# guenthermi/postgres-word2vec

Measured on AMD Instinct MI355X. Metric: batched IVFADC kNN queries/sec (k=5) + recall@5, 3Mx300d, higher is better.
Workload: dtype f32; 1 GPU; IVFADC batch (ivfadc_batch_search generalised to nprobe), 3000000x300d, C=1000, m=12, K=1024, nprobe=10, k=5, batch=1024 queries per GPU, replicated index, queries sharded by rank; N=3000000, d=300, C=1000, m=12, K=1024, nprobe=10, k=5, batch_per_gpu=1024, parallelism=dp1, world_size=1, backend=none (single GPU), batches_in_flight=4

## Files before the change

### postgres-word2vec_amd/csrc/fused5.h

```cpp
#pragma once
#include <hip/hip_runtime.h>
#include <stdint.h>

#include "refine.h"
#include "coarse.h"
#include "scan_tail5.h"

namespace freddy {

static constexpr int SCAN5_G = 16;

__host__ __device__ __forceinline__ constexpr int filt5_bias(int p, int m) { return FILT5_VMAX + (p < 32768 - FILT5_VMAX * m ? 1 : 0); }
__device__ __forceinline__ uint32_t lane_byte4() {
  uint32_t x;
  asm volatile("v_mbcnt_lo_u32_b32 %0, -1, 0\n\tv_mbcnt_hi_u32_b32 %0, -1, %0\n\tv_lshlrev_b32 %0, 2, %0" : "=v"(x));
  return x;
}
typedef short s2v __attribute__((ext_vector_type(2)));
__device__ __forceinline__ uint32_t pk_add_i16(uint32_t x, uint32_t y) {
  return __builtin_bit_cast(uint32_t, __builtin_bit_cast(s2v, x) + __builtin_bit_cast(s2v, y));
}

template <int S, int QT>
__device__ __forceinline__ void query_codebook5_body(const float* __restrict__ queries, const float* __restrict__ cbT,
                                                     const float* __restrict__ cmax, float* __restrict__ qn,
                                                     float* __restrict__ qscale, uint32_t* __restrict__ qc,
                                                     int Q, int d, int m, int K, int bx, int by, unsigned char* smem,
                                                     uint32_t* __restrict__ qc8 = nullptr) {
  static_assert(QT == 16, "one 16-lane group per query");
  constexpr int SP = (S + 3) & ~3;
  float (*qs)[SP] = reinterpret_cast<float (*)[SP]>(smem);
  float* inv_s = reinterpret_cast<float*>(smem + QT * SP * 4);
  const int tid = threadIdx.x, p = bx, q0 = by * QT;
  constexpr int STEPS_B = (S + 3) / 4;
  float bv[STEPS_B][4][2];
  auto load_b = [&](int g) {
    typedef float f4b __attribute__((ext_vector_type(4)));
    const f4b* src = reinterpret_cast<const f4b*>(cbT + ((((size_t)p * 8 + g) * STEPS_B) * 64 + (tid & 63)) * 8);
#pragma unroll
    for (int st = 0; st < STEPS_B; ++st) {
      const f4b lo = src[(size_t)st * 128], hi = src[(size_t)st * 128 + 1];
      bv[st][0][0] = lo.x; bv[st][0][1] = lo.y; bv[st][1][0] = lo.z; bv[st][1][1] = lo.w;
      bv[st][2][0] = hi.x; bv[st][2][1] = hi.y; bv[st][3][0] = hi.z; bv[st][3][1] = hi.w;
    }
  };
  load_b((tid >> 6) * 2);
  for (int i = tid; i < QT * SP; i += 256) {
    const int qi = i / SP, j = i - qi * SP;
    qs[qi][j] = (j < S && q0 + qi < Q) ? queries[(size_t)(q0 + qi) * d + p * S + j] : 0.0f;
  }
  {
    const int qi = tid >> 4, pp = tid & 15, q = q0 + qi;
    float best = 0.0f;
    if (pp < m && q < Q) {
      float n2 = 0.0f;
      for (int j = 0; j < S; ++j) { const float v = queries[(size_t)q * d + pp * S + j]; n2 = __builtin_fmaf(v, v, n2); }
      const float nrm = __builtin_sqrtf(n2) * (1.0f + 1e-5f);
      if (p == 0) qn[(size_t)q * m + pp] = nrm;
      best = 2.0f * nrm * cmax[pp];
    }
#pragma unroll
    for (int o = 8; o > 0; o >>= 1) best = fmaxf(best, __shfl_xor(best, o, 64));
    if (pp == 0) {
      const float sc = q < Q ? best * (1.0f / (float)FILT5_VMAX) * (1.0f + 1e-6f) : 0.0f;
      inv_s[qi] = (sc > 0.0f && sc < 1e30f) ? 1.0f / sc : 0.0f;
      if (p == 0 && q < Q) qscale[q] = sc;
    }
  }
  {
    typedef float f4v __attribute__((ext_vector_type(4)));
    __syncthreads();
    const int wave = tid >> 6, lane = tid & 63, col = lane & 15, kq = lane >> 4;
    const int nq = (Q - q0 < QT) ? Q - q0 : QT;
    constexpr int STEPS = (S + 3) / 4;
    float av[STEPS];
#pragma unroll
    for (int st = 0; st < STEPS; ++st) av[st] = 4 * st + kq < S ? qs[col][4 * st + kq] : 0.0f;
    const float vmax = (float)FILT5_VMAX;
    const int bias = filt5_bias(p, m);
#pragma unroll
    for (int gg = 0; gg < 2; ++gg) {
      const int g = wave * 2 + gg;
      f4v acc[4][2];
#pragma unroll
      for (int i = 0; i < 4; ++i) acc[i][0] = acc[i][1] = f4v{0.0f, 0.0f, 0.0f, 0.0f};
#pragma unroll
      for (int st = 0; st < STEPS; ++st)
#pragma unroll
        for (int i = 0; i < 4; ++i)
#pragma unroll
          for (int e = 0; e < 2; ++e) acc[i][e] = __builtin_amdgcn_mfma_f32_16x16x4f32(av[st], bv[st][i][e], acc[i][e], 0, 0, 0);
      if (gg == 0) load_b(g + 1);
#pragma unroll
      for (int reg = 0; reg < 4; ++reg) {
        const int qi = 4 * kq + reg;
        if (qi < nq) {
          const float inv = inv_s[qi];
          uint32_t wd[4];
#pragma unroll
          for (int i = 0; i < 4; ++i) {
            const int i0 = (int)fminf(fmaxf(__builtin_rintf(-2.0f * acc[i][0][reg] * inv), -vmax), vmax) + bias;
            const int i1 = (int)fminf(fmaxf(__builtin_rintf(-2.0f * acc[i][1][reg] * inv), -vmax), vmax) + bias;
            wd[i] = (uint32_t)i0 | ((uint32_t)i1 << 16);
          }
          *reinterpret_cast<uint4*>(qc + ((size_t)(q0 + qi) * m + p) * 512 + 4 * (16 * g + col)) = uint4{wd[0], wd[1], wd[2], wd[3]};
          if (qc8) qc8[((size_t)(q0 + qi) * m + p) * 128 + (16 * g + col)] = (wd[0] & 0xffffu) | (wd[1] << 16);
        }
      }
    }
  }
}
template <int S, int QT>
static constexpr int query_codebook5_lds() { return QT * ((S + 3) & ~3) * 4 + QT * 4; }
template <int S, int QT>
__global__ __launch_bounds__(256) void query_codebook5_kernel(const float* __restrict__ queries, const float* __restrict__ cbT,
                                                             const float* __restrict__ cmax, float* __restrict__ qn,
                                                             float* __restrict__ qscale, uint32_t* __restrict__ qc,
                                                             int Q, int d, int m, int K, uint32_t* __restrict__ qc8) {
  __shared__ __attribute__((aligned(16))) unsigned char smem[query_codebook5_lds<S, QT>()];
  query_codebook5_body<S, QT>(queries, cbT, cmax, qn, qscale, qc, Q, d, m, K, blockIdx.x, blockIdx.y, smem, qc8);
}

struct CoarseTableArgs {
  const float* queries;
  const float* coarseF; const float* cn2; float* dist; float* qn2; int Q, Cpad, d, dp; ZeroArgs z; int coarse_gx, coarse_gy;
  const float* cbT; const float* cmax; float* qn; float* qscale; uint32_t* qc; int m, K;
  float* tmin; int C;
  const ch8v* coarseH; int ec;
  uint32_t* qc8;
};
template <int S, int QT, bool H16 = false>
__global__ __launch_bounds__(256) void coarse_table5_kernel(CoarseTableArgs a) {
  extern __shared__ __attribute__((aligned(16))) unsigned char smem[];
  const int n_coarse = a.coarse_gx * a.coarse_gy;
  const int b = blockIdx.x;
  if (b < n_coarse) {
    if constexpr (H16)
      coarse_approx16_body(a.queries, a.coarseH, a.ec, a.cn2, a.dist, a.qn2, a.Q, a.Cpad, a.d, a.z, b % a.coarse_gx, b / a.coarse_gx,
                           a.coarse_gx, a.coarse_gy, smem, a.tmin, a.C);
    else
    coarse_approx_body(a.queries, a.coarseF, a.cn2, a.dist, a.qn2, a.Q, a.Cpad, a.d, a.dp, a.z, b % a.coarse_gx, b / a.coarse_gx,
                       a.coarse_gx, a.coarse_gy, smem, a.tmin, a.C);
  } else {
    const int t = b - n_coarse;
    query_codebook5_body<S, QT>(a.queries, a.cbT, a.cmax, a.qn, a.qscale, a.qc, a.Q, a.d, a.m, a.K, t % a.m, t / a.m, smem, a.qc8);
  }
}

template <int M>
__global__ __launch_bounds__(256) void entry_record5_kernel(RecordArgs a) {
  const int lane = threadIdx.x & 63;
  const int e = blockIdx.x * 4 + (threadIdx.x >> 6);
  if (a.elastic && blockIdx.x == 0 && threadIdx.x == 0) __hip_atomic_fetch_add(a.elastic + EL_PENDING, a.n_announce, FREDDY_RLX_AGENT);
  if (e >= a.n_groups[0]) return;
  const int cell = a.group_cell[e], first = a.group_first[e], gc = a.group_cnt[e];
  const int cnt = gc & 0xff, chunk = gc >> 8;
  int32_t* rec = a.records + (size_t)e * REC_DW;
  if (lane == 0) {
    const int b0 = a.blk_off[cell] + chunk * FUSED_UNIT_BLOCKS;
    int nb = a.blk_off[cell + 1] - b0;
    if (nb > FUSED_UNIT_BLOCKS) nb = FUSED_UNIT_BLOCKS;
    int rows = a.list_off[cell + 1] - a.list_off[cell] - chunk * (FUSED_UNIT_BLOCKS * 64);
    if (rows > FUSED_UNIT_BLOCKS * 64) rows = FUSED_UNIT_BLOCKS * 64;
    rec[0] = cell; rec[1] = cnt; rec[2] = chunk; rec[3] = b0; rec[4] = nb; rec[5] = rows;
  }
  if (lane < 16) {
    const int it = lane < cnt ? a.sorted_item[first + lane] : -1;
    const int q = a.item_query[it >= 0 ? it : a.sorted_item[first]];
    const float sc = a.qscale[q];
    ItemBounds ib = item_bounds(0.0f, 0.0f, a.sentinel);
    if (it >= 0) ib = item_bounds(a.item_dist[it], filter_width5<M>(a.qn + (size_t)q * M, a.pmax, sc), a.sentinel);
    rec[8 + lane] = it;
    rec[24 + lane] = q;
    rec[40 + lane] = (int32_t)__float_as_uint(ib.off);
    rec[56 + lane] = (int32_t)__float_as_uint(ib.e);
    rec[72 + lane] = (int32_t)__float_as_uint(ib.shift);
    rec[88 + lane] = (int32_t)ib.lo_bits;
    rec[104 + lane] = (int32_t)ib.hi_bits;
    rec[128 + lane] = (int32_t)__float_as_uint((it >= 0 && sc < 1e30f) ? sc : 0.0f);
    const float A = it >= 0 ? a.item_dist[it] : -1.0f;
    const bool fin = it >= 0 && ib.e < 1e30f && A >= 0.0f && A < 1e30f;
    rec[144 + lane] = (int32_t)__float_as_uint(fin ? A * (1.0f + 2e-5f) : __uint_as_float(0x7f800000u));
    rec[160 + lane] = (int32_t)__float_as_uint(fin ? A * (1.0f - 2e-5f) : 0.0f);
  }
}

template <int M, bool FULLK, bool CAND, bool PROF, bool U8, bool ELASTIC>
__device__ __forceinline__ void ivf_filter5_body(const FilterArgs& a) {
  static_assert(!(U8 && FULLK), "one byte per code: K <= 256");
  constexpr int G = SCAN5_G, RMAX = FUSED_RMAX, NG = SPEC2_NG;
  constexpr int NP = M / 2;
  constexpr int ROWB = G * 2;
  constexpr int HROWB = 16;
  static_assert(M == 12 && G == 16 && SPEC2_NB == 8, "layout");
  typedef uint32_t u2 __attribute__((ext_vector_type(2)));
  typedef uint32_t u4 __attribute__((ext_vector_type(4)));
  extern __shared__ __attribute__((aligned(16))) unsigned char smem[];
  unsigned char* slab = smem;
  uint32_t* colmin = reinterpret_cast<uint32_t*>(smem + a.desc_offset);
  uint32_t* thr_s = colmin + 16 * 64;
  int32_t* dsc = reinterpret_cast<int32_t*>(smem + a.desc_offset + 4096 + 64);
  int32_t* gidq = dsc + 2 * REC_DW;
  float* rt_s = reinterpret_cast<float*>(gidq + 4);

  const int tid = threadIdx.x, lane = tid & 63;
  const int wave = __builtin_amdgcn_readfirstlane(tid >> 6);
  const bool builder = wave < SPEC2_NB;
  const int K = FULLK ? 1024 : a.K;
  const uint32_t HALFB = (uint32_t)K * HROWB;
  const uint32_t POSB = 2u * HALFB;
  const uint32_t BUFB = 2u * POSB;
  const int n_work = a.n_groups[0];

  int cur = 0, ei = 0;
  const int n_own = ELASTIC ? a.n_own : (int)gridDim.x;
  const bool extra = ELASTIC && (int)blockIdx.x >= n_own;
  if (!extra) {
    if (tid == 0) {
      gidq[0] = (int)blockIdx.x; gidq[1] = n_own + atomicAdd(a.work_counter, 1);
      if constexpr (ELASTIC) {
        __hip_atomic_fetch_sub(a.elastic + EL_PENDING, 1, FREDDY_RLX_AGENT);
        if ((int)blockIdx.x < n_work) __hip_atomic_fetch_add(a.elastic + EL_ACTIVE, 1, FREDDY_RLX_AGENT);
      }
    }
    if (tid < REC_DW) dsc[tid] = a.records[(size_t)blockIdx.x * REC_DW + tid];
  } else if (tid == 0) {
    const int pend = __hip_atomic_load(a.elastic + EL_PENDING, FREDDY_RLX_AGENT);
    const int claims = __hip_atomic_load(a.work_counter, FREDDY_RLX_AGENT);
    const int alive = __hip_atomic_fetch_add(a.elastic + EL_ACTIVE, 1, FREDDY_RLX_AGENT);
    int g = -1;
    if (pend - (claims < n_own ? n_own - claims : 0) <= 0 && alive < a.cap) g = n_own + atomicAdd(a.work_counter, 1);
    if (g < 0 || g >= n_work) {
      g = -1;
      __hip_atomic_fetch_sub(a.elastic + EL_ACTIVE, 1, FREDDY_RLX_AGENT);
    } else {
      __hip_atomic_fetch_add(a.elastic + EL_STARTED, 1, FREDDY_RLX_AGENT);
    }
    const bool leave = g >= 0 && a.elastic_yield == 2;
    if (leave) __hip_atomic_fetch_add(a.elastic + EL_YIELDED, 1, FREDDY_RLX_AGENT);
    gidq[0] = g; gidq[1] = (leave || g < 0) ? 0x7fffffff : n_own + atomicAdd(a.work_counter, 1); gidq[2] = leave ? 1 : 0;
  }
  for (int i = tid; i < 16 * 64; i += SPEC2_T) colmin[i] = 0xffffffffu;
  __syncthreads();
  if (extra) {
    const int first = __builtin_amdgcn_readfirstlane(gidq[0]);
    if (first < 0) return;
    if (tid < REC_DW) dsc[tid] = a.records[(size_t)first * REC_DW + tid];
    __syncthreads();
  } else if ((int)blockIdx.x >= n_work) return;

  if (builder) {
    const int hpos = (wave >> 1) & 1;
    const int half = wave >> 2;
    const int li = (wave & 1) * 64 + lane;
    const uint32_t qoff = (uint32_t)hpos * POSB + (uint32_t)half * HALFB + (uint32_t)li * HROWB;
    const uint32_t vq = (uint32_t)li * 16u + (uint32_t)hpos * 2048u;
    u4 qw[2][8];
#pragma unroll
    for (int s = 0; s < 2; ++s)
#pragma unroll
      for (int g = 0; g < 8; ++g) qw[s][g] = u4{0u, 0u, 0u, 0u};
    typedef const char __attribute__((address_space(1))) * gptrc;
    typedef const u4 __attribute__((address_space(1))) * gptr4u;
    auto issue = [&](int set, int phase, const int (&qids)[8], int nh) {
      if (half >= nh || (a.fence & 32)) return;
      uint32_t voff = vq + (uint32_t)phase * 4096u;
      asm volatile("" : "+v"(voff));
#pragma unroll
      for (int u = 0; u < 8; ++u) {
        const gptrc qb = (gptrc)(uintptr_t)a.qc + (size_t)(uint32_t)qids[u] * (size_t)(M * 2048);
        qw[set][u] = *(gptr4u)(qb + voff);
      }
    };
    auto emit = [&](int set, unsigned char* dst, int nh) {
      if (half >= nh || (a.fence & 16)) return;
      unsigned char* dp = dst + qoff;
#pragma unroll
      for (int k = 0; k < 4; ++k) {
        uint32_t w[8];
#pragma unroll
        for (int u = 0; u < 8; ++u)
          w[u] = k == 0 ? qw[set][u].x : k == 1 ? qw[set][u].y : k == 2 ? qw[set][u].z : qw[set][u].w;
        const u4 lo = u4{__builtin_amdgcn_perm(w[1], w[0], 0x05040100u), __builtin_amdgcn_perm(w[3], w[2], 0x05040100u),
                         __builtin_amdgcn_perm(w[5], w[4], 0x05040100u), __builtin_amdgcn_perm(w[7], w[6], 0x05040100u)};
        const u4 hi = u4{__builtin_amdgcn_perm(w[1], w[0], 0x07060302u), __builtin_amdgcn_perm(w[3], w[2], 0x07060302u),
// ... 265 lines not shown
```

### postgres-word2vec_amd/csrc/pin.hip

```cpp
#include "internal.h"

#include "kernels.h"
#include "scan_common.h"
#include "coarse.h"
#include "mutate.h"

static std::vector<float> transpose_codebook(const float* cb, int m, int K, int S) {
  std::vector<float> t((size_t)m * S * K);
  for (int p = 0; p < m; ++p)
    for (int c = 0; c < K; ++c)
      for (int j = 0; j < S; ++j) t[((size_t)p * S + j) * K + c] = cb[((size_t)p * K + c) * S + j];
  return t;
}

static void arrange_list_rows(const int16_t* codes, int m, int64_t lo, int64_t hi, std::vector<int64_t>& order) {
  const int64_t n = hi - lo;
  order.resize((size_t)n);
  for (int64_t i = 0; i < n; ++i) order[(size_t)i] = lo + i;
  if (n <= 16 || m > 16) return;
  static const int WINDOW = (int)env_int("FREDDY_GPU_ARRANGE_WINDOW", 1024);
  int cnt[16][16], mx[16];
  for (int64_t k = 0; k < n; ++k) {
    if ((k & 15) == 0) { memset(cnt, 0, sizeof(cnt)); memset(mx, 0, sizeof(mx)); }
    const int64_t wend = std::min<int64_t>(n, k + WINDOW);
    int64_t best = k;
    int best_cost = INT32_MAX;
    for (int64_t j = k; j < wend; ++j) {
      const int16_t* row = codes + (size_t)order[(size_t)j] * m;
      int cost = 0;
      for (int p = 0; p < m; ++p) {
        const int c = cnt[p][row[p] & 15];
        cost += c + (c + 1 > mx[p] ? 100 : 0);
      }
      if (cost < best_cost) { best_cost = cost; best = j; }
    }
    std::swap(order[(size_t)k], order[(size_t)best]);
    const int16_t* row = codes + (size_t)order[(size_t)k] * m;
    for (int p = 0; p < m; ++p) {
      const int c = ++cnt[p][row[p] & 15];
      if (c > mx[p]) mx[p] = c;
    }
  }
  static const int GROUP_LANES[64] = {0,  1,  2,  3,  12, 13, 14, 15, 20, 21, 22, 23, 24, 25, 26, 27, 4,  5,  6,  7,  8,  9,
                                      10, 11, 16, 17, 18, 19, 28, 29, 30, 31, 32, 33, 34, 35, 44, 45, 46, 47, 52, 53, 54, 55,
                                      56, 57, 58, 59, 36, 37, 38, 39, 40, 41, 42, 43, 48, 49, 50, 51, 60, 61, 62, 63};
  std::vector<int64_t> blk(64);
  for (int64_t b0 = 0; b0 + 64 <= n; b0 += 64) {
    for (int j = 0; j < 64; ++j) blk[(size_t)GROUP_LANES[j]] = order[(size_t)(b0 + j)];
    for (int j = 0; j < 64; ++j) order[(size_t)(b0 + j)] = blk[(size_t)j];
  }
}

static int pack_lists(freddy_gpu_index* ix, int n_lists, const int32_t* list_off, const int16_t* codes,
                      const int32_t* row_pos ) {
  const int m = ix->m, K = ix->K, M2 = ix->M2;
  BlockPlan plan;
  int bad = 0;
  if (const int why = plan_blocks(n_lists, [&](int c) { return (int64_t)list_off[c + 1] - list_off[c]; }, plan, &bad))
    return why == PLAN_NEGATIVE_LENGTH ? fail(FREDDY_E_ARG, "list_off is not non-decreasing at list %d", bad) : fail(FREDDY_E_LIMIT, "N too large for 32-bit row positions");
  const std::vector<int32_t>& blk_off = plan.blk_off;
  const int64_t n_blocks = plan.n_blocks;
  std::vector<uint32_t> packed((size_t)alloc_blocks(n_blocks) * M2 * 64, 0u);
  std::vector<int32_t> pos((size_t)alloc_blocks(n_blocks) * 64, -1);
  const bool arrange = row_pos != nullptr;
  std::vector<std::vector<int64_t>> orders(arrange ? (size_t)n_lists : 0);
  if (arrange) {
    std::atomic<int> next_list{0};
    auto worker = [&]() {
      for (int c = next_list.fetch_add(1); c < n_lists; c = next_list.fetch_add(1))
        arrange_list_rows(codes, m, list_off[c], list_off[c + 1], orders[(size_t)c]);
    };
    const unsigned nt = std::max(1u, std::min(32u, std::thread::hardware_concurrency()));
    std::vector<std::thread> pool;
    for (unsigned t = 1; t < nt && (int)t < n_lists; ++t) pool.emplace_back(worker);
    worker();
    for (auto& th : pool) th.join();
  }
  for (int c = 0; c < n_lists; ++c) {
    for (int64_t i = 0; i < (int64_t)list_off[c + 1] - list_off[c]; ++i) {
      const int64_t r = arrange ? orders[(size_t)c][(size_t)i] : list_off[c] + i;
      const int64_t b = blk_off[c] + i / 64;
      const int lane = (int)(i % 64);
      const int16_t* row = codes + (size_t)r * m;
      for (int l = 0; l < m; ++l) {
        if (row[l] < 0 || row[l] >= K)
          return fail(FREDDY_E_ARG, "code %d at row %lld position %d is outside [0,%d)", (int)row[l],
                      (long long)r, l, K);
      }
      for (int j = 0; j < M2; ++j) {
        const uint32_t lo = (uint16_t)row[2 * j];
        const uint32_t hi = (2 * j + 1 < m) ? (uint16_t)row[2 * j + 1] : 0u;
        packed[((size_t)b * M2 + j) * 64 + lane] = lo | (hi << 16);
      }
      pos[(size_t)b * 64 + lane] = row_pos ? row_pos[r] : (int32_t)r;
    }
  }
  if (upload(&ix->blk_cell, plan.blk_cell.data(), plan.blk_cell.size(), &ix->bytes))
    return fail(FREDDY_E_NOMEM, "device allocation/copy failed while pinning the lists");
  ix->n_blocks = n_blocks;
  ix->max_list_blocks = plan.max_list_blocks;
  ix->h_list_off.assign(list_off, list_off + n_lists + 1);
  if (upload(&ix->blk_off, blk_off.data(), blk_off.size(), &ix->bytes) ||
      upload(&ix->list_off, list_off, (size_t)n_lists + 1, &ix->bytes) ||
      upload(&ix->packed, packed.data(), packed.size(), &ix->bytes) ||
      upload(&ix->pos, pos.data(), pos.size(), &ix->bytes))
    return fail(FREDDY_E_NOMEM, "device allocation/copy failed while pinning the lists");
  return 0;
}

__global__ __launch_bounds__(256) void pack8_kernel(const uint32_t* __restrict__ packed, uint32_t* __restrict__ packed8, int64_t n_blocks) {
  const int64_t i = (int64_t)blockIdx.x * 256 + threadIdx.x;
  if (i >= n_blocks * 3 * 64) return;
  const int lane = (int)(i & 63);
  const int64_t bt = i >> 6;
  const int t = (int)(bt % 3);
  const int64_t b = bt / 3;
  const uint32_t p0 = packed[((size_t)b * 6 + 2 * t) * 64 + lane], p1 = packed[((size_t)b * 6 + 2 * t + 1) * 64 + lane];
  packed8[i] = (p0 & 0xffu) | (((p0 >> 16) & 0xffu) << 8) | ((p1 & 0xffu) << 16) | (((p1 >> 16) & 0xffu) << 24);
}
static int make_packed8(const freddy_gpu_index* ix, const uint32_t* packed, int64_t n_blocks, uint32_t** out, int64_t* out_bytes) {
  *out = nullptr; *out_bytes = 0;
  if (ix->K > 256 || ix->m != 12 || ix->M2 != 6 || !packed || n_blocks <= 0) return 0;
  const size_t bytes = sizeof(uint32_t) * (size_t)n_blocks * 3 * 64;
  if (dev_malloc(out, bytes) != hipSuccess) { *out = nullptr; return fail(FREDDY_E_NOMEM, "device allocation of %zu bytes failed (one-byte codes)", bytes); }
  const int64_t n = n_blocks * 3 * 64;
  hipLaunchKernelGGL(pack8_kernel, dim3((unsigned)((n + 255) / 256)), dim3(256), 0, ix->stream, packed, *out, n_blocks);
  if (hipGetLastError() != hipSuccess || hipStreamSynchronize(ix->stream) != hipSuccess) {
    (void)dev_free(*out); *out = nullptr;
    return fail(FREDDY_E_HIP, "building the one-byte codes failed");
  }
  *out_bytes = (int64_t)bytes;
  return 0;
}
static void install_packed8(freddy_gpu_index* ix, uint32_t* p8, int64_t bytes) {
  if (ix->packed8 && ix->packed8_own) { (void)dev_free(ix->packed8); ix->bytes -= ix->packed8_bytes; }
  ix->packed8 = p8; ix->packed8_own = p8 != nullptr; ix->packed8_bytes = bytes;
  ix->bytes += bytes;
}
static int build_packed8(freddy_gpu_index* ix) {
  uint32_t* p8 = nullptr;
  int64_t bytes = 0;
  if (int rc = make_packed8(ix, ix->packed, ix->n_blocks, &p8, &bytes)) return rc;
  install_packed8(ix, p8, bytes);
  return 0;
}

static int derive_codebook_tables_into(freddy_gpu_index* ix, const float* codebook);
static int make_row_terms(const freddy_gpu_index* ix, const uint32_t* packed, const int32_t* blk_cell, int64_t n_blocks, const float* cbR, float** out, int64_t* out_bytes);
static void install_row_terms(freddy_gpu_index* ix, float* rterm, int64_t bytes);
static int derive_codebook_tables(freddy_gpu_index* ix, const float* codebook, bool with_row_terms = false) {
  float* const old[] = {ix->cbT, ix->cbP, ix->cbR, ix->pmax, ix->cmaxp, ix->cbF};
  const int64_t bytes_before = ix->bytes;
  ix->cbT = ix->cbP = ix->cbR = ix->pmax = ix->cmaxp = ix->cbF = nullptr;
  int rc = derive_codebook_tables_into(ix, codebook);
  float* rterm = nullptr;
  int64_t rterm_bytes = 0;
  if (!rc && with_row_terms) rc = make_row_terms(ix, ix->packed, ix->blk_cell, ix->n_blocks, ix->cbR, &rterm, &rterm_bytes);
  if (rc) {
    float* const fresh[] = {ix->cbT, ix->cbP, ix->cbR, ix->pmax, ix->cmaxp, ix->cbF};
    for (float* p : fresh) if (p) (void)dev_free(p);
    ix->cbT = old[0]; ix->cbP = old[1]; ix->cbR = old[2]; ix->pmax = old[3]; ix->cmaxp = old[4]; ix->cbF = old[5];
    ix->bytes = bytes_before;
    return rc;
  }
  if (with_row_terms) install_row_terms(ix, rterm, rterm_bytes);
  int64_t old_bytes = 0;
  if (old[0]) old_bytes += (int64_t)sizeof(float) * ix->m * ix->S * ix->K;
  if (old[1]) old_bytes += (int64_t)sizeof(float) * ix->m * (((ix->S + 3) & ~3) / 4) * FUSED_T * 8;
  if (old[2]) old_bytes += (int64_t)sizeof(float) * ix->m * ix->K * ix->S;
  if (old[3]) old_bytes += (int64_t)sizeof(float) * ix->m;
  if (old[4]) old_bytes += (int64_t)sizeof(float) * ix->m;
  if (old[5]) old_bytes += (int64_t)sizeof(float) * ix->m * 8 * 7 * 64 * 8;
  ix->bytes -= old_bytes;
  for (float* p : old) if (p) (void)dev_free(p);
  if (ix->kind == KIND_PQ) drop_pq_views(ix);
  return 0;
}
static int build_fragment_codebook(freddy_gpu_index* ix, const float* codebook) {
  std::vector<float> f((size_t)ix->m * 8 * 7 * 64 * 8, 0.0f);
  for (int p = 0; p < ix->m; ++p)
    for (int g = 0; g < 8; ++g)
      for (int st = 0; st < 7; ++st)
        for (int l = 0; l < 64; ++l)
          for (int i = 0; i < 4; ++i)
            for (int e = 0; e < 2; ++e) {
              const int j = 4 * st + (l >> 4), c = 128 * i + 16 * g + (l & 15) + 512 * e;
              if (j < ix->S && c < ix->K)
                f[((((size_t)p * 8 + g) * 7 + st) * 64 + l) * 8 + i * 2 + e] = codebook[((size_t)p * ix->K + c) * ix->S + j];
            }
  if (upload(&ix->cbF, f.data(), f.size(), &ix->bytes)) return fail(FREDDY_E_NOMEM, "device allocation failed");
  return 0;
}
static inline double norm_max(double a, double b) { return (b != b || b > a) ? b : a; }
static int derive_codebook_tables_into(freddy_gpu_index* ix, const float* codebook) {
  std::vector<float> cbT = transpose_codebook(codebook, ix->m, ix->K, ix->S);
  if (upload(&ix->cbT, cbT.data(), cbT.size(), &ix->bytes)) return fail(FREDDY_E_NOMEM, "device allocation failed");
  if (ix->kind == KIND_PQ) {
    if (ix->m == 12 && ix->S == 25 && ix->K <= FUSED_T * FUSED_E) {
      std::vector<float> cmaxp((size_t)ix->m);
      for (int p = 0; p < ix->m; ++p) {
        double cmax = 0.0;
        for (int c = 0; c < ix->K; ++c) {
          double n2 = 0.0;
          for (int j = 0; j < ix->S; ++j) { const double v = codebook[((size_t)p * ix->K + c) * ix->S + j]; n2 += v * v; }
          cmax = norm_max(cmax, std::sqrt(n2));
        }
        cmaxp[p] = (float)(cmax * (1.0 + 1e-6));
      }
      if (upload(&ix->cbR, codebook, (size_t)ix->m * ix->K * ix->S, &ix->bytes) ||
          upload(&ix->pmax, cmaxp.data(), cmaxp.size(), &ix->bytes) ||
          upload(&ix->cmaxp, cmaxp.data(), cmaxp.size(), &ix->bytes))
        return fail(FREDDY_E_NOMEM, "device allocation failed");
      if (int rc = build_fragment_codebook(ix, codebook)) return rc;
    }
    return 0;
  }
  if (ix->kind != KIND_IVF) return 0;
  const int C = ix->C, d = ix->d;
  if (ix->K <= FUSED_T * FUSED_E) {
    const int SP = (ix->S + 3) & ~3, SPq = SP / 4;
    std::vector<float> cbP((size_t)ix->m * SPq * FUSED_T * 8, 0.0f);
    for (int p = 0; p < ix->m; ++p)
      for (int jb = 0; jb < SPq; ++jb)
        for (int tl = 0; tl < FUSED_T; ++tl)
          for (int u = 0; u < 4; ++u)
            for (int e = 0; e < 2; ++e) {
              const int j = jb * 4 + u, c = tl + e * FUSED_T;
              if (j < ix->S && c < ix->K)
                cbP[((((size_t)p * SPq + jb) * FUSED_T + tl) * 4 + u) * 2 + e] = codebook[((size_t)p * ix->K + c) * ix->S + j];
            }
    if (upload(&ix->cbP, cbP.data(), cbP.size(), &ix->bytes)) return fail(FREDDY_E_NOMEM, "device allocation failed");
  }
  if (ix->cbP && ix->m == 12 && ix->S == 25) {
    std::vector<float> pmax((size_t)ix->m), cmaxp((size_t)ix->m);
    for (int p = 0; p < ix->m; ++p) {
      double comax = 0.0, cmax = 0.0;
      for (int c = 0; c < C; ++c) {
        double n2 = 0.0;
        for (int j = 0; j < ix->S; ++j) { const double v = ix->h_coarse[(size_t)c * d + p * ix->S + j]; n2 += v * v; }
        comax = norm_max(comax, std::sqrt(n2));
      }
      for (int c = 0; c < ix->K; ++c) {
        double n2 = 0.0;
        for (int j = 0; j < ix->S; ++j) { const double v = codebook[((size_t)p * ix->K + c) * ix->S + j]; n2 += v * v; }
        cmax = norm_max(cmax, std::sqrt(n2));
      }
      pmax[p] = (float)((comax + cmax) * (1.0 + 1e-6));
      cmaxp[p] = (float)(cmax * (1.0 + 1e-6));
    }
    if (upload(&ix->cbR, codebook, (size_t)ix->m * ix->K * ix->S, &ix->bytes) ||
        upload(&ix->pmax, pmax.data(), pmax.size(), &ix->bytes) ||
        upload(&ix->cmaxp, cmaxp.data(), cmaxp.size(), &ix->bytes))
      return fail(FREDDY_E_NOMEM, "device allocation failed");
    if (int rc = build_fragment_codebook(ix, codebook)) return rc;
  }
  return 0;
}

static int make_row_terms(const freddy_gpu_index* ix, const uint32_t* packed, const int32_t* blk_cell, int64_t n_blocks, const float* cbR, float** out, int64_t* out_bytes) {
  *out = nullptr; *out_bytes = 0;
  if (!cbR) return 0;
  const int64_t n_slots = alloc_blocks(n_blocks) * 64;
  if (dev_malloc(out, sizeof(float) * (size_t)n_slots) != hipSuccess) { *out = nullptr; return fail(FREDDY_E_NOMEM, "device allocation failed (row terms)"); }
  if (n_blocks > 0) {
    hipLaunchKernelGGL(row_term_kernel, dim3((unsigned)((n_blocks * 64 + 255) / 256)), dim3(256), 0, ix->stream, packed,
                       blk_cell, ix->coarse, cbR, *out, n_blocks * 64, ix->M2, ix->d, ix->m, ix->K, ix->S);
    if (hipGetLastError() != hipSuccess || hipStreamSynchronize(ix->stream) != hipSuccess) {
      (void)dev_free(*out); *out = nullptr;
      return fail(FREDDY_E_HIP, "building the row terms failed");
    }
  }
  *out_bytes = (int64_t)sizeof(float) * n_slots;
  return 0;
}
static void install_row_terms(freddy_gpu_index* ix, float* rterm, int64_t bytes) {
  if (ix->rterm) (void)dev_free(ix->rterm);
  ix->bytes += bytes - ix->rterm_bytes;
  ix->rterm = rterm; ix->rterm_bytes = bytes;
}
static int refresh_row_terms(freddy_gpu_index* ix) {
  float* rterm = nullptr;
  int64_t bytes = 0;
  if (int rc = make_row_terms(ix, ix->packed, ix->blk_cell, ix->n_blocks, ix->cbR, &rterm, &bytes)) return rc;
  install_row_terms(ix, rterm, bytes);
  return 0;
}

static int raise_lds_limits(int device) {
  static std::mutex mu;
  static std::vector<char> done;
  std::lock_guard<std::mutex> g(mu);
  if ((size_t)device < done.size() && done[(size_t)device]) return 0;
  for (const std::vector<LdsLimit>& unit : {lds_limits_ivfadc(), lds_limits_pq(), lds_limits_join(), lds_limits_exact()})
    for (const LdsLimit& l : unit) HIP_TRY(hipFuncSetAttribute(l.kernel, hipFuncAttributeMaxDynamicSharedMemorySize, l.bytes));
  if (done.size() <= (size_t)device) done.resize((size_t)device + 1, 0);
  done[(size_t)device] = 1;
  return 0;
}

int open_device(freddy_gpu_index* ix, int device) {
  if (!ix->registered) { ix->registered = true; backend_handles(+1, device); }
  choose_hw_queues(device);
  int n = 0;
  HIP_TRY(hipGetDeviceCount(&n));
  if (device < 0 || device >= n) return fail(FREDDY_E_ARG, "device %d out of range (%d visible)", device, n);
  HIP_TRY(hipSetDevice(device));
  ix->device = device;
  ix->tune = read_tuning();
  if (int rc = raise_lds_limits(device)) return rc;
  HIP_TRY(hipStreamCreateWithFlags(&ix->stream, hipStreamNonBlocking));
  hipDeviceProp_t prop;
  if (hipGetDeviceProperties(&prop, device) == hipSuccess && prop.multiProcessorCount > 0) ix->n_cus = ix->device_cus = prop.multiProcessorCount;
  return 0;
}

static int check_pq_shape(int d, int m, int K, int64_t N) {
  if (d <= 0 || m <= 0 || K <= 0 || N < 0) return fail(FREDDY_E_ARG, "non-positive dimension");
  if (d % m) return fail(FREDDY_E_ARG, "d=%d is not a multiple of m=%d", d, m);
  if (K > 65536) return fail(FREDDY_E_LIMIT, "K=%d does not fit a 16-bit code", K);
  if ((size_t)m * K * 4 + 4096 > 160 * 1024)
    return fail(FREDDY_E_LIMIT, "LUT of m*K=%d floats does not fit the 160 KiB LDS", m * K);
  if (N > (int64_t)INT32_MAX - 64) return fail(FREDDY_E_LIMIT, "N too large for 32-bit row positions");
  return 0;
}

extern "C" int freddy_gpu_pin_pq(const freddy_pq_desc* t, int device, freddy_gpu_index_t** out) {
  if (!t || !out || !t->codebook || (t->N && (!t->ids || !t->codes))) return fail(FREDDY_E_ARG, "NULL argument");
  if (int rc = check_pq_shape(t->d, t->m, t->K, t->N)) return rc;
  for (int64_t r = 1; r < t->N; ++r)
    if (t->ids[r] <= t->ids[r - 1])
      return fail(FREDDY_E_ARG, "ids must be strictly ascending (canonical scan order); violated at row %lld", (long long)r);
  freddy_gpu_index* ix = new freddy_gpu_index();
  ix->kind = KIND_PQ;
  ix->d = t->d; ix->m = t->m; ix->K = t->K; ix->S = t->d / t->m; ix->M2 = (t->m + 1) / 2; ix->N = t->N;
  int rc = open_device(ix, device);
  if (!rc) rc = derive_codebook_tables(ix, t->codebook);
  if (!rc && upload(&ix->ids, t->ids, (size_t)t->N, &ix->bytes)) rc = fail(FREDDY_E_NOMEM, "device allocation failed");
  if (!rc) {
    const int32_t off[2] = {0, (int32_t)t->N};
    rc = pack_lists(ix, 1, off, t->codes, nullptr);
    if (!rc) rc = build_packed8(ix);
  }
  if (!rc) { ix->h_ids.assign(t->ids, t->ids + t->N); ix->max_id = t->N ? t->ids[t->N - 1] : -1; }
// ... 147 lines not shown
```

### postgres-word2vec_amd/csrc/refine.h

```cpp
#pragma once
#include <hip/hip_runtime.h>
#include <stdint.h>

#include "scan_common.h"
#include "fused3.h"

namespace freddy {

struct FilterArgs {
  const uint32_t* qc;
  const float* rterm;
  const int32_t* records;
  const int32_t* n_groups;
  int32_t* work_counter;
  const uint32_t* packed;
  u64* surv;
  int32_t* surv_count;
  int32_t* cand_count;
  int K, L, upi;
  float sentinel;
  uint32_t desc_offset;
  uint32_t fence;
  int keep_all;
  long long* prof;
  const uint32_t* packed8;
  uint32_t* tau_run;
  const uint32_t* qc8;
  int Lt;
  int32_t* elastic;
  int n_own, cap, elastic_yield;
};
enum { EL_ACTIVE = 0, EL_PENDING = 1, EL_STARTED = 2, EL_YIELDED = 3 };
#define FREDDY_RLX_AGENT __ATOMIC_RELAXED, __HIP_MEMORY_SCOPE_AGENT

static constexpr int FILT5_VMAX = 2730;
static constexpr float FILT5_EPS = 512.0f * 5.9604644775390625e-8f * 1.0001f;
template <int M>
__device__ __forceinline__ float filter_width5(const float* __restrict__ qn, const float* __restrict__ pmax, float scale) {
  float sb = 0.0f;
#pragma unroll
  for (int p = 0; p < M; ++p) {
    const float t = qn[p] + pmax[p];
    sb = __builtin_fmaf(t, t, sb);
  }
  return __builtin_fmaf(sb, FILT5_EPS, __builtin_fmaf(28.0f, scale, 1e-30f));
}

struct ItemBounds {
  float off;
  float e;
  float shift;
  uint32_t lo_bits;
  uint32_t hi_bits;
};
__device__ __forceinline__ ItemBounds item_bounds(float A, float E, float sentinel) {
  ItemBounds b;
  if (E < 1e30f && A < 1e30f && A >= 0.0f) {
    const float a_up = A * (1.0f + 2e-5f), a_lo = A * (1.0f - 2e-5f);
    b.off = a_up + E;
    b.e = E;
    b.shift = ((b.off - a_lo) + 0.25f * E) * (1.0f + 1e-6f);
    const float hi = (sentinel + b.shift) * (1.0f + 1e-6f);
    const float lo = ((sentinel + b.shift) - E) * (1.0f - 1e-6f);
    b.hi_bits = hi < 3e38f ? __float_as_uint(hi) : 0xfffffffeu;
    b.lo_bits = lo > 0.0f ? __float_as_uint(lo < 3e38f ? lo : 3e38f) : 0u;
  } else {
    b.off = 0.0f;
    b.e = __uint_as_float(0x7f800000u);
    b.shift = __uint_as_float(0x7f800000u);
    b.lo_bits = 0u;
    b.hi_bits = 0xfffffffeu;
  }
  return b;
}
__device__ __forceinline__ uint32_t widen_threshold(uint32_t tau_bits, float E) {
  if (tau_bits >= 0x7f800000u || !(E < 1e30f)) return 0xfffffffeu;
  const float t = (__uint_as_float(tau_bits) + E) * (1.0f + 2.4e-7f);
  return __float_as_uint(t);
}

static __global__ __launch_bounds__(256) void row_term_kernel(const uint32_t* __restrict__ packed, const int32_t* __restrict__ blk_cell,
                                                      const float* __restrict__ coarse, const float* __restrict__ cbR,
                                                      float* __restrict__ rterm, int64_t n_slots, int M2, int d, int m, int K, int S) {
  const int64_t slot = (int64_t)blockIdx.x * 256 + threadIdx.x;
  if (slot >= n_slots) return;
  const int64_t block = slot >> 6;
  const int lane = (int)(slot & 63);
  const int cell = blk_cell[block];
  double acc = 0.0;
  for (int p = 0; p < m; ++p) {
    const uint32_t word = packed[((size_t)block * M2 + (p >> 1)) * 64 + lane];
    const int code = (int)((word >> ((p & 1) * 16)) & 0xffffu);
    const float* cv = cbR + ((size_t)p * K + (code < K ? code : 0)) * S;
    const float* co = coarse + (size_t)cell * d + (size_t)p * S;
    for (int j = 0; j < S; ++j) acc += (double)cv[j] * (double)cv[j] + 2.0 * (double)co[j] * (double)cv[j];
  }
  rterm[slot] = (float)acc;
}

static constexpr int REC_DW = 176;

struct RecordArgs {
  const int32_t* group_cell;
  const int32_t* group_first;
  const int32_t* group_cnt;
  const int32_t* n_groups;
  const int32_t* sorted_item;
  const int32_t* item_query;
  const int32_t* blk_off;
  const int32_t* list_off;
  const float* item_dist;
  const float* qn;
  const float* qscale;
  const float* pmax;
  int32_t* records;
  float sentinel;
  int32_t* elastic;
  int n_announce;
};

struct MergeRefineArgs {
  const u64* surv;
  const int32_t* surv_count;
  const int32_t* active;
  const int32_t* round_rows;
  const int32_t* item_cell;
  const float* queries;
  const float* coarse;
  const float* cbR;
  const float* qn;
  const float* pmax;
  const float* qscale5;
  const uint32_t* packed;
  const int32_t* pos;
  const int32_t* blk_cell;
  int32_t* cand_count;
  int32_t* violations;
  int32_t* out_ids;
  float* out_dist;
  int32_t* found;
  int32_t* next_active;
  int32_t* n_next;
  int32_t* status;
  int n_active, W, upi, L, k, found_rule, first_round, K, d;
  float sentinel;
  int refine_all;
  uint32_t fence;
  int slices;
  u64* part;
};

template <int S, int M, int NWV, bool MANY = false, bool PARTIAL = false>
__global__ __launch_bounds__(64 * NWV, 4) void merge_refine_kernel(MergeRefineArgs a) {
  static_assert(!MANY || NWV > 1, "the split selection needs the four waves");
  static_assert(!PARTIAL || MANY, "slices of a query: the flat PQ table's instantiation");
  constexpr int NT = NWV > 4 ? NWV : 4;
  static_assert(NT * 64 / M <= 64, "a round's rows are finalised by one wave");
  constexpr int NC = NT * 64 / M;
  constexpr int SQ = S + 1;
  constexpr int M2 = M / 2;
  __shared__ u64 stage_all[MANY ? NWV : 1][64];
  u64* const stage = stage_all[0];
  __shared__ u64 part_key[MANY ? NWV : 1][MANY ? 64 : 1];
  __shared__ uint32_t part_flag[MANY ? NWV : 1][MANY ? 64 : 1];
  __shared__ float qs[M * S];
  __shared__ float sq[NWV == 1 ? 32 * SQ : NT * 64 * SQ];
  __shared__ float lutv[NT * 64];
  __shared__ int32_t cbo[NT * 64], coo[NT * 64];
  __shared__ u64 cq_key[64 + NC];
  __shared__ int32_t cq_cell[64 + NC];
  __shared__ int sh_n;
  constexpr int BQ = MANY ? 512 : 1;
  __shared__ u64 bq_key[BQ];
  constexpr int PB = 256;
  __shared__ int pref_all[MANY ? NWV : 1][PB + 1];
  __shared__ int bq_n;
  __shared__ uint32_t sh_T;
  const int x = blockIdx.x, lane = threadIdx.x & 63;
  const int wave = __builtin_amdgcn_readfirstlane((int)(threadIdx.x >> 6));
  const int q = PARTIAL ? x / a.slices : (a.active ? a.active[x] : x);
  const int k = a.k;
  const int per_item = a.upi * FUSED_NW;
  const int R = a.W * per_item;
  constexpr int NBATCH = 4;

  if (!(a.fence & 2)) for (int j = threadIdx.x; j < M * S; j += 64 * NWV) qs[j] = a.queries[(size_t)q * a.d + j];
  const float E = (a.fence & 2) ? 0.0f : filter_width5<M>(a.qn + (size_t)q * M, a.pmax, a.qscale5[q]);

  auto tile_work = [&](int t, float* sqb, int n) {
// ... 362 lines not shown
```

Measured before the change: 11.99 million queries/s.

## Compute query-codebook table with split-fp16 MFMA instead of fp32 MFMA

Replaces the fp32 16x16x4 MFMA loop (7 k-steps per output tile) in the query-codebook table kernel with three 16x16x32 fp16 MFMAs per tile. Queries and codebook are each split into hi and lo fp16 parts with per-position power-of-two exponent scaling, and the results are unscaled with ldexp. The host-side fragment codebook is rebuilt as hi/lo fp16 halves with stored exponents. It also adds a waves_per_eu(4) occupancy hint to the table kernels. The aim is fewer matrix instructions and less codebook load traffic, at the cost of dropping the lo*lo term, which could slightly perturb the quantized table values.

```diff
diff --git a/postgres-word2vec_amd/csrc/fused5.h b/postgres-word2vec_amd/csrc/fused5.h
--- a/postgres-word2vec_amd/csrc/fused5.h
+++ b/postgres-word2vec_amd/csrc/fused5.h
@@ -32,19 +32,15 @@
   float (*qs)[SP] = reinterpret_cast<float (*)[SP]>(smem);
   float* inv_s = reinterpret_cast<float*>(smem + QT * SP * 4);
   const int tid = threadIdx.x, p = bx, q0 = by * QT;
-  constexpr int STEPS_B = (S + 3) / 4;
-  float bv[STEPS_B][4][2];
+  static_assert(S <= 32 && SP % 4 == 0, "one k-step of v_mfma_f32_16x16x32_f16 covers a position");
+  ch8v bh[8], bl[8];
   auto load_b = [&](int g) {
-    typedef float f4b __attribute__((ext_vector_type(4)));
-    const f4b* src = reinterpret_cast<const f4b*>(cbT + ((((size_t)p * 8 + g) * STEPS_B) * 64 + (tid & 63)) * 8);
-#pragma unroll
-    for (int st = 0; st < STEPS_B; ++st) {
-      const f4b lo = src[(size_t)st * 128], hi = src[(size_t)st * 128 + 1];
-      bv[st][0][0] = lo.x; bv[st][0][1] = lo.y; bv[st][1][0] = lo.z; bv[st][1][1] = lo.w;
-      bv[st][2][0] = hi.x; bv[st][2][1] = hi.y; bv[st][3][0] = hi.z; bv[st][3][1] = hi.w;
-    }
+    const ch8v* src = reinterpret_cast<const ch8v*>(cbT) + ((size_t)p * 8 + g) * (CBF_GROUP_HALVES / 8) + (tid & 63);
+#pragma unroll
+    for (int t = 0; t < 8; ++t) { bh[t] = src[(size_t)t * 128]; bl[t] = src[(size_t)t * 128 + 64]; }
   };
   load_b((tid >> 6) * 2);
+  const int ecb = reinterpret_cast<const int*>(cbT)[cbf_exp_offset(m) + p];
   for (int i = tid; i < QT * SP; i += 256) {
     const int qi = i / SP, j = i - qi * SP;
     qs[qi][j] = (j < S && q0 + qi < Q) ? queries[(size_t)(q0 + qi) * d + p * S + j] : 0.0f;
@@ -72,10 +68,30 @@
     __syncthreads();
     const int wave = tid >> 6, lane = tid & 63, col = lane & 15, kq = lane >> 4;
     const int nq = (Q - q0 < QT) ? Q - q0 : QT;
-    constexpr int STEPS = (S + 3) / 4;
-    float av[STEPS];
-#pragma unroll
-    for (int st = 0; st < STEPS; ++st) av[st] = 4 * st + kq < S ? qs[col][4 * st + kq] : 0.0f;
+    ch8v ah, al;
+    int eq = 0;
+    {
+      f4v x0 = f4v{0.0f, 0.0f, 0.0f, 0.0f}, x1 = x0;
+      if (8 * kq < SP) x0 = *reinterpret_cast<const f4v*>(&qs[col][8 * kq]);
+      if (8 * kq + 4 < SP) x1 = *reinterpret_cast<const f4v*>(&qs[col][8 * kq + 4]);
+      const float x[8] = {x0.x, x0.y, x0.z, x0.w, x1.x, x1.y, x1.z, x1.w};
+      float am = 0.0f;
+#pragma unroll
+      for (int j = 0; j < 8; ++j) am = fmaxf(am, __builtin_fabsf(x[j]));
+      am = fmaxf(am, __shfl_xor(am, 16, 64));
+      am = fmaxf(am, __shfl_xor(am, 32, 64));
+      if (am > 0.0f && am < 3e38f) { (void)__builtin_frexpf(am, &eq); eq = CBF_EXP - eq; }
+#pragma unroll
+      for (int j = 0; j < 8; ++j) {
+        const float v = __builtin_ldexpf(x[j], eq);
+        const _Float16 hh = (_Float16)v;
+        ah[j] = hh;
+        al[j] = (_Float16)(v - (float)hh);
+      }
+    }
+    int unscale[4];
+#pragma unroll
+    for (int reg = 0; reg < 4; ++reg) unscale[reg] = -(__shfl(eq, 4 * kq + reg, 64) + ecb);
     const float vmax = (float)FILT5_VMAX;
     const int bias = filt5_bias(p, m);
 #pragma unroll
@@ -83,13 +99,17 @@
       const int g = wave * 2 + gg;
       f4v acc[4][2];
 #pragma unroll
-      for (int i = 0; i < 4; ++i) acc[i][0] = acc[i][1] = f4v{0.0f, 0.0f, 0.0f, 0.0f};
-#pragma unroll
-      for (int st = 0; st < STEPS; ++st)
-#pragma unroll
-        for (int i = 0; i < 4; ++i)
-#pragma unroll
-          for (int e = 0; e < 2; ++e) acc[i][e] = __builtin_amdgcn_mfma_f32_16x16x4f32(av[st], bv[st][i][e], acc[i][e], 0, 0, 0);
+      for (int i = 0; i < 4; ++i)
+#pragma unroll
+        for (int e = 0; e < 2; ++e) acc[i][e] = __builtin_amdgcn_mfma_f32_16x16x32_f16(al, bh[2 * i + e], f4v{0.0f, 0.0f, 0.0f, 0.0f}, 0, 0, 0);
+#pragma unroll
+      for (int i = 0; i < 4; ++i)
+#pragma unroll
+        for (int e = 0; e < 2; ++e) acc[i][e] = __builtin_amdgcn_mfma_f32_16x16x32_f16(ah, bl[2 * i + e], acc[i][e], 0, 0, 0);
+#pragma unroll
+      for (int i = 0; i < 4; ++i)
+#pragma unroll
+        for (int e = 0; e < 2; ++e) acc[i][e] = __builtin_amdgcn_mfma_f32_16x16x32_f16(ah, bh[2 * i + e], acc[i][e], 0, 0, 0);
       if (gg == 0) load_b(g + 1);
 #pragma unroll
       for (int reg = 0; reg < 4; ++reg) {
@@ -99,8 +119,8 @@
           uint32_t wd[4];
 #pragma unroll
           for (int i = 0; i < 4; ++i) {
-            const int i0 = (int)fminf(fmaxf(__builtin_rintf(-2.0f * acc[i][0][reg] * inv), -vmax), vmax) + bias;
-            const int i1 = (int)fminf(fmaxf(__builtin_rintf(-2.0f * acc[i][1][reg] * inv), -vmax), vmax) + bias;
+            const int i0 = (int)fminf(fmaxf(__builtin_rintf(-2.0f * __builtin_ldexpf(acc[i][0][reg], unscale[reg]) * inv), -vmax), vmax) + bias;
+            const int i1 = (int)fminf(fmaxf(__builtin_rintf(-2.0f * __builtin_ldexpf(acc[i][1][reg], unscale[reg]) * inv), -vmax), vmax) + bias;
             wd[i] = (uint32_t)i0 | ((uint32_t)i1 << 16);
           }
           *reinterpret_cast<uint4*>(qc + ((size_t)(q0 + qi) * m + p) * 512 + 4 * (16 * g + col)) = uint4{wd[0], wd[1], wd[2], wd[3]};
@@ -110,10 +130,11 @@
     }
   }
 }
+#define FREDDY_TABLE_UNIT_KERNEL __global__ __launch_bounds__(256) __attribute__((amdgpu_waves_per_eu(4)))
 template <int S, int QT>
 static constexpr int query_codebook5_lds() { return QT * ((S + 3) & ~3) * 4 + QT * 4; }
 template <int S, int QT>
-__global__ __launch_bounds__(256) void query_codebook5_kernel(const float* __restrict__ queries, const float* __restrict__ cbT,
+FREDDY_TABLE_UNIT_KERNEL void query_codebook5_kernel(const float* __restrict__ queries, const float* __restrict__ cbT,
                                                              const float* __restrict__ cmax, float* __restrict__ qn,
                                                              float* __restrict__ qscale, uint32_t* __restrict__ qc,
                                                              int Q, int d, int m, int K, uint32_t* __restrict__ qc8) {
@@ -130,7 +151,7 @@
   uint32_t* qc8;
 };
 template <int S, int QT, bool H16 = false>
-__global__ __launch_bounds__(256) void coarse_table5_kernel(CoarseTableArgs a) {
+FREDDY_TABLE_UNIT_KERNEL void coarse_table5_kernel(CoarseTableArgs a) {
   extern __shared__ __attribute__((aligned(16))) unsigned char smem[];
   const int n_coarse = a.coarse_gx * a.coarse_gy;
   const int b = blockIdx.x;
diff --git a/postgres-word2vec_amd/csrc/pin.hip b/postgres-word2vec_amd/csrc/pin.hip
--- a/postgres-word2vec_amd/csrc/pin.hip
+++ b/postgres-word2vec_amd/csrc/pin.hip
@@ -170,25 +170,46 @@
   if (old[2]) old_bytes += (int64_t)sizeof(float) * ix->m * ix->K * ix->S;
   if (old[3]) old_bytes += (int64_t)sizeof(float) * ix->m;
   if (old[4]) old_bytes += (int64_t)sizeof(float) * ix->m;
-  if (old[5]) old_bytes += (int64_t)sizeof(float) * ix->m * 8 * 7 * 64 * 8;
+  if (old[5]) old_bytes += (int64_t)sizeof(float) * (int64_t)cbf_floats(ix->m);
   ix->bytes -= old_bytes;
   for (float* p : old) if (p) (void)dev_free(p);
   if (ix->kind == KIND_PQ) drop_pq_views(ix);
   return 0;
 }
 static int build_fragment_codebook(freddy_gpu_index* ix, const float* codebook) {
-  std::vector<float> f((size_t)ix->m * 8 * 7 * 64 * 8, 0.0f);
-  for (int p = 0; p < ix->m; ++p)
+  static_assert(sizeof(_Float16) == 2 && sizeof(float) == 4 && sizeof(int32_t) == 4, "layout");
+  if (ix->S > 32) return fail(FREDDY_E_ARG, "table kernel: more than 32 dimensions per position");
+  std::vector<_Float16> f(2 * cbf_floats(ix->m), (_Float16)0.0f);
+  _Float16* h = f.data();
+  for (int p = 0; p < ix->m; ++p) {
+    float amax = 0.0f;
+    for (size_t i = 0; i < (size_t)ix->K * ix->S; ++i) {
+      const float v = std::fabs(codebook[(size_t)p * ix->K * ix->S + i]);
+      if (v < 3e38f && v > amax) amax = v;
+    }
+    int32_t ecb = 0;
+    if (amax > 0.0f) { int e = 0; (void)frexpf(amax, &e); ecb = CBF_EXP - e; }
+    std::memcpy(h + 2 * (cbf_exp_offset(ix->m) + p), &ecb, 4);
     for (int g = 0; g < 8; ++g)
-      for (int st = 0; st < 7; ++st)
-        for (int l = 0; l < 64; ++l)
-          for (int i = 0; i < 4; ++i)
-            for (int e = 0; e < 2; ++e) {
-              const int j = 4 * st + (l >> 4), c = 128 * i + 16 * g + (l & 15) + 512 * e;
-              if (j < ix->S && c < ix->K)
-                f[((((size_t)p * 8 + g) * 7 + st) * 64 + l) * 8 + i * 2 + e] = codebook[((size_t)p * ix->K + c) * ix->S + j];
-            }
-  if (upload(&ix->cbF, f.data(), f.size(), &ix->bytes)) return fail(FREDDY_E_NOMEM, "device allocation failed");
+      for (int t = 0; t < 8; ++t)
+        for (int l = 0; l < 64; ++l) {
+          const int c = 128 * (t >> 1) + 16 * g + (l & 15) + 512 * (t & 1);
+          if (c >= ix->K) continue;
+          _Float16* hi = h + ((size_t)p * 8 + g) * CBF_GROUP_HALVES + ((size_t)(t * 2) * 64 + l) * 8;
+          _Float16* lo = hi + 64 * 8;
+          for (int u = 0; u < 8; ++u) {
+            const int j = 8 * (l >> 4) + u;
+            if (j >= ix->S) continue;
+            const float v = ldexpf(codebook[((size_t)p * ix->K + c) * ix->S + j], ecb);
+            hi[u] = (_Float16)v;
+            lo[u] = (_Float16)(v - (float)hi[u]);
+          }
+        }
+  }
+  _Float16* dF = nullptr;
+  const int up = upload(&dF, f.data(), f.size(), &ix->bytes);
+  ix->cbF = reinterpret_cast<float*>(dF);
+  if (up) return fail(FREDDY_E_NOMEM, "device allocation failed");
   return 0;
 }
 static inline double norm_max(double a, double b) { return (b != b || b > a) ? b : a; }
diff --git a/postgres-word2vec_amd/csrc/refine.h b/postgres-word2vec_amd/csrc/refine.h
--- a/postgres-word2vec_amd/csrc/refine.h
+++ b/postgres-word2vec_amd/csrc/refine.h
@@ -35,6 +35,10 @@
 
 static constexpr int FILT5_VMAX = 2730;
 static constexpr float FILT5_EPS = 512.0f * 5.9604644775390625e-8f * 1.0001f;
+static constexpr int CBF_EXP = 10;
+static constexpr size_t CBF_GROUP_HALVES = 8 * 2 * 64 * 8;
+__host__ __device__ constexpr size_t cbf_exp_offset(int m) { return (size_t)m * 8 * CBF_GROUP_HALVES / 2; }
+__host__ __device__ constexpr size_t cbf_floats(int m) { return cbf_exp_offset(m) + (size_t)m; }
 template <int M>
 __device__ __forceinline__ float filter_width5(const float* __restrict__ qn, const float* __restrict__ pmax, float scale) {
   float sb = 0.0f;
```

Measured after the change: 12.38 million queries/s, median of 6. +3.3%, better.
